# phaistos-networks/Trinity

Hardware: NVIDIA H100
Metric: queries/sec (batched 2-term AND, 100M-doc Zipfian synthetic index) (higher is better)
Workload: dtype u32

## Files before the change

### include/trinity_b200.h

```cpp
#ifndef TRINITY_B200_H
#define TRINITY_B200_H
#include <stddef.h>
#include <stdint.h>

#ifdef __cplusplus
extern "C" {
#endif

#define TRN_OK 0
#define TRN_ERR_ARG (-1)
#define TRN_ERR_CUDA (-2)
#define TRN_ERR_FORMAT (-3)
#define TRN_ERR_STATE (-4)
#define TRN_ERR_PARSE (-5)
#define TRN_ERR_CAPACITY (-6)
#define TRN_ERR_UNSUPPORTED (-7)

#define TRN_CODEC_GOOGLE 0
#define TRN_CODEC_LUCENE 1

typedef struct trn_term {
        uint32_t documents;
        uint32_t chunk_off;
        uint32_t chunk_len;
// ... 95 lines not shown

int         trn_create(int device, trn_ctx **out);
void        trn_destroy(trn_ctx *);
const char *trn_last_error(trn_ctx *);
int trn_set_stream(trn_ctx *, void *cuda_stream);

int trn_upload_index(trn_ctx *, int codec, const uint8_t *index, uint64_t nbytes, const trn_term *terms, uint32_t nterms, uint32_t max_docid);

int trn_set_masked_documents(trn_ctx *, const uint32_t *docids, uint64_t n);

typedef struct trn_index_info {
        int      codec;
        uint32_t nterms, max_docid, tile_docs, ntiles, block_docs;
        uint64_t index_bytes, directory_bytes, total_blocks, total_postings;
        uint64_t dense_terms, dense_bitmap_bytes;
} trn_index_info;
int trn_index_info_get(trn_ctx *, trn_index_info *out);

int trn_upload_hits(trn_ctx *, const uint8_t *index, uint64_t nbytes, const uint8_t *hits, uint64_t hits_bytes);

#define TRN_MODE_DOCS_ONLY 0
#define TRN_MODE_SCORED_ALL 1
#define TRN_MODE_SCORED_TOPK 2
#define TRN_MODE_DOCS_COMPACT 3

typedef struct trn_result {
        uint32_t        nq;
        uint64_t        total;
        const uint64_t *offsets;
        const uint32_t *docids;
// ... 43 lines not shown
#define TRN_ROUTE_CANDIDATE 3
#define TRN_ROUTE_SCORE_FLAT 4
#define TRN_ROUTE_FLAT_TREE 5
#define TRN_ROUTE_EXEC_TILES 6
int trn_debug_last_routes(trn_ctx *, uint8_t *out, uint32_t cap, uint32_t *n);
int trn_debug_plan(int codec, const uint8_t *index, uint64_t nbytes, const trn_term *terms, uint32_t nterms, uint32_t max_docid, const trn_query *queries,
                   uint32_t nq, int mode, uint32_t k, uint8_t *routes, uint32_t *nslots, char *err, size_t errcap);
int trn_debug_dense_runs(int codec, const uint8_t *index, uint64_t nbytes, const trn_term *terms, uint32_t nterms, uint32_t max_docid, const trn_query *queries,
                         uint32_t nq, int mode, uint32_t k, uint32_t *qtiles, uint32_t *tickets, uint64_t cap, uint64_t *n, char *err, size_t errcap);
int trn_debug_mixed_runs(int codec, const uint8_t *index, uint64_t nbytes, const trn_term *terms, uint32_t nterms, uint32_t max_docid, const trn_query *queries,
                         uint32_t nq, int mode, uint32_t k, uint32_t *qtiles, uint32_t *tickets, uint64_t cap, uint64_t *n, char *err, size_t errcap);
int trn_debug_cand_runs(int codec, const uint8_t *index, uint64_t nbytes, const trn_term *terms, uint32_t nterms, uint32_t max_docid, const trn_query *queries,
                        uint32_t nq, int mode, uint32_t k, uint32_t *qtiles, uint32_t *tickets, uint64_t cap, uint64_t *n, char *err, size_t errcap);

int trn_debug_dense_terms(int codec, const uint8_t *index, uint64_t nbytes, const trn_term *terms, uint32_t nterms, uint32_t *offsets, uint32_t *nselected,
                          uint64_t *bitmap_bytes, char *err, size_t errcap);

int trn_debug_dense_bitmap(trn_ctx *, uint32_t term, uint32_t *out, uint64_t cap, uint64_t *base, uint64_t *nwords);

#define TRN_MODE_MATCHED_TERMS 4
typedef struct trn_hit {
        uint64_t payload;
        uint16_t pos;
        uint8_t  payload_len;
} trn_hit;
typedef struct trn_matches {
        uint32_t        nq;
        uint64_t        total_matches, total_terms, total_hits;
        const uint64_t *doc_offsets;
        const uint32_t *docids;
// ... 163 lines not shown
```

### trinity_b200/__init__.py

```python
from __future__ import annotations

import ctypes as C
import os
from dataclasses import dataclass
from typing import Iterable, List, Optional, Sequence

import numpy as np

from ._ffi import (HIT_DTYPE, QNODE_DTYPE, TERM_DTYPE, TrnIndexInfo, TrnIntersections, TrnIsectReq, TrnMatches, TrnPercolation, TrnPercolatorInfo, TrnQuery,
                   TrnIndexed, TrnMerged, TrnMergeSource, TrnResult, TrnTerm, TrnTimings, lib)

CODEC_GOOGLE, CODEC_LUCENE = 0, 1
MODE_DOCS_ONLY, MODE_SCORED_ALL, MODE_SCORED_TOPK = 0, 1, 2
MODE_MATCHED_TERMS = 4
MODE_DOCS_COMPACT = 3
NODE_TERM, NODE_AND, NODE_OR, NODE_NOT, NODE_OPTIONAL, NODE_SOME, NODE_PHRASE = 0, 1, 2, 3, 4, 5, 6
ROUTE_STEPS, ROUTE_FLAT_AND, ROUTE_FLAT_OR, ROUTE_CANDIDATE, ROUTE_SCORE_FLAT, ROUTE_FLAT_TREE, ROUTE_EXEC_TILES = 0, 1, 2, 3, 4, 5, 6
EMPTY_TERM = 0xFFFFFFFF
DENSE_NONE = 0xFFFFFFFF
DOC_IDS_END = 0xFFFFFFFF
DOCSET_NONE = 0xFFFFFFFF


class TrinityError(RuntimeError):
# ... 277 lines not shown
    arr, keep = _pack_queries(queries)
    qtiles = np.zeros((max(len(queries), 1), 2), np.uint32)
    n = C.c_uint64()
    err = C.create_string_buffer(256)
    args = (codec, _ptr(index), index.size, _ptr(terms), len(terms), max_docid, C.cast(arr, C.c_void_p), len(queries), mode, k, _ptr(qtiles))
    rc = fn(*args, None, 0, C.byref(n), err, 256)
    tickets = np.zeros((max(n.value, 1), 3), np.uint32)
    if rc == -6:
        rc = fn(*args, _ptr(tickets), n.value, C.byref(n), err, 256)
    if rc != 0:
        raise TrinityError(err.value.decode("utf-8", "replace") or f"rc={rc}")
    return qtiles[: len(queries)].copy(), tickets[: n.value].copy()


def debug_dense_terms(codec: int, index: np.ndarray, terms: np.ndarray):
    index = np.ascontiguousarray(index, dtype=np.uint8)
    terms = np.ascontiguousarray(terms, dtype=TERM_DTYPE)
    off = np.zeros(max(len(terms), 1), np.uint32)
    n, nbytes = C.c_uint32(), C.c_uint64()
    err = C.create_string_buffer(256)
    rc = lib().trn_debug_dense_terms(codec, _ptr(index), index.size, _ptr(terms), len(terms), _ptr(off), C.byref(n), C.byref(nbytes), err, 256)
    if rc != 0:
        raise TrinityError(err.value.decode("utf-8", "replace") or f"rc={rc}")
    off = off[: len(terms)].copy()
    assert int(np.count_nonzero(off != DENSE_NONE)) == n.value
    return off, int(nbytes.value)


def bm25_idf(doc_freq: int, docs_cnt: int) -> float:
    return float(lib().trn_bm25_idf(doc_freq, docs_cnt))


def bm25_score(idf: float, freq: int) -> float:
    return float(lib().trn_bm25_score(idf, freq))


@dataclass
class BatchResult:
    nq: int
    mode: int
    k: int
# ... 788 lines not shown
```

### trinity_b200/_ffi.py

```python
from __future__ import annotations

import ctypes as C
from pathlib import Path

import numpy as np

_LIB_PATH = Path(__file__).resolve().parent / "libtrinity_b200.so"

EXPORTS = [
    "trn_builder_create", "trn_builder_destroy", "trn_builder_begin_term", "trn_builder_begin_document",
    "trn_builder_new_hit", "trn_builder_end_document", "trn_builder_end_term", "trn_builder_add_term",
    "trn_builder_set_google_skiplist_countdown", "trn_builder_index", "trn_builder_hits", "trn_builder_last_error",
    "trn_synth_build", "trn_synth_build_shard", "trn_synth_build_ex", "trn_builder_set_google_block", "trn_synth_destroy", "trn_synth_index", "trn_synth_hits", "trn_synth_terms", "trn_synth_sum_hits",
    "trn_synth_postings", "trn_synth_positions",
    "trn_directory_probe", "trn_directory_stats", "trn_directory_lookup", "trn_dict_create", "trn_dict_destroy", "trn_parse_query_dict", "trn_segment_open", "trn_segment_close", "trn_segment_info", "trn_segment_index", "trn_segment_terms",
    "trn_segment_masked", "trn_parse_query", "trn_query_truth_table", "trn_debug_compile", "trn_bm25_idf", "trn_bm25_score",
    "trn_create", "trn_destroy", "trn_last_error", "trn_set_stream", "trn_upload_index", "trn_set_masked_documents", "trn_index_info_get",
    "trn_exec_batch", "trn_exec_batch_device", "trn_last_topk_device", "trn_merge_topk", "trn_fetch_results", "trn_last_timings",
    "trn_decode_terms", "trn_result_for_each", "trn_result_decode", "trn_upload_hits", "trn_debug_positions", "trn_encode_google", "trn_encode_lucene", "trn_debug_chunk_plan",
    "trn_encode_google_payloads", "trn_encode_lucene_payloads", "trn_index_documents_payloads",
    "trn_debug_last_routes", "trn_debug_plan", "trn_debug_dense_runs", "trn_debug_mixed_runs", "trn_debug_cand_runs", "trn_debug_dense_terms", "trn_debug_dense_bitmap",
    "trn_exec_matches", "trn_debug_hits", "trn_intersect", "trn_debug_intersect_plan",
    "trn_percolator_register", "trn_percolate", "trn_debug_percolator_plan",
    "trn_index_documents", "trn_segment_write", "trn_merge_sources", "trn_merge_sources_payloads", "trn_debug_merge_plan",
    "trn_docset_create", "trn_docset_destroy", "trn_exec_batch_filtered", "trn_exec_batch_device_filtered", "trn_exec_matches_filtered",
]

TERM_DTYPE = np.dtype([("documents", "<u4"), ("chunk_off", "<u4"), ("chunk_len", "<u4")])
QNODE_DTYPE = np.dtype([("kind", "u1"), ("nchildren", "u1"), ("first_child", "<u2"), ("term", "<u4"), ("weight", "<f8")])
STEP_DTYPE = np.dtype([("op", "u1"), ("mode", "u1"), ("dst", "u1"), ("src", "u1"), ("flags", "u1"), ("pad", "u1", (3,)), ("term", "<u4"), ("pad2", "<u4"), ("idf", "<f8")])
assert TERM_DTYPE.itemsize == 12 and QNODE_DTYPE.itemsize == 16 and STEP_DTYPE.itemsize == 24


class TrnTerm(C.Structure):
    _fields_ = [("documents", C.c_uint32), ("chunk_off", C.c_uint32), ("chunk_len", C.c_uint32)]


class TrnQuery(C.Structure):
    _fields_ = [("nodes", C.c_void_p), ("nnodes", C.c_uint32), ("root", C.c_uint32)]


class TrnIndexInfo(C.Structure):
    _fields_ = [("codec", C.c_int), ("nterms", C.c_uint32), ("max_docid", C.c_uint32), ("tile_docs", C.c_uint32),
                ("ntiles", C.c_uint32), ("block_docs", C.c_uint32), ("index_bytes", C.c_uint64), ("directory_bytes", C.c_uint64),
                ("total_blocks", C.c_uint64), ("total_postings", C.c_uint64), ("dense_terms", C.c_uint64), ("dense_bitmap_bytes", C.c_uint64)]


class TrnResult(C.Structure):
    _fields_ = [("nq", C.c_uint32), ("total", C.c_uint64), ("offsets", C.POINTER(C.c_uint64)),
                ("docids", C.POINTER(C.c_uint32)), ("scores", C.POINTER(C.c_float)),
                ("match_counts", C.POINTER(C.c_uint64)), ("postings_scanned", C.c_uint64),
                ("index_bytes_touched", C.c_uint64), ("kernel_launches", C.c_uint32), ("device_ms", C.c_float), ("exec_kernel_ms", C.c_float),
                ("words", C.POINTER(C.c_uint32)), ("total_words", C.c_uint64), ("item_desc", C.POINTER(C.c_uint32)), ("qitems", C.c_void_p)]


HIT_DTYPE = np.dtype({"names": ["payload", "pos", "payload_len"], "formats": ["<u8", "<u2", "u1"], "offsets": [0, 8, 10], "itemsize": 16})


class TrnMatches(C.Structure):
    _fields_ = [("nq", C.c_uint32), ("total_matches", C.c_uint64), ("total_terms", C.c_uint64), ("total_hits", C.c_uint64),
# ... 138 lines not shown
    sig("trn_encode_lucene_payloads", i32, vp, vp, u32, vp, vp, vp, vp, vp, vp, C.c_uint64, P(C.c_uint64), vp, C.c_uint64, P(C.c_uint64), vp, P(C.c_float))
    sig("trn_debug_last_routes", i32, vp, vp, u32, P(u32))
    sig("trn_exec_matches", i32, vp, vp, u32, P(TrnMatches))
    sig("trn_docset_create", i32, vp, vp, u64, P(u32))
    sig("trn_docset_destroy", i32, vp, u32)
    sig("trn_exec_batch_filtered", i32, vp, vp, u32, i32, u32, vp, P(TrnResult))
    sig("trn_exec_batch_device_filtered", i32, vp, vp, u32, i32, u32, vp, P(TrnResult))
    sig("trn_exec_matches_filtered", i32, vp, vp, u32, vp, P(TrnMatches))
    sig("trn_debug_hits", i32, i32, vp, C.c_uint64, vp, C.c_uint64, vp, vp, u32, vp, vp, vp, C.c_uint64, P(C.c_uint64), C.c_char_p, C.c_size_t)
    sig("trn_debug_plan", i32, i32, vp, u64, vp, u32, u32, vp, u32, i32, u32, vp, P(u32), C.c_char_p, C.c_size_t)
    sig("trn_debug_dense_runs", i32, i32, vp, u64, vp, u32, u32, vp, u32, i32, u32, vp, vp, u64, P(u64), C.c_char_p, C.c_size_t)
    sig("trn_debug_mixed_runs", i32, i32, vp, u64, vp, u32, u32, vp, u32, i32, u32, vp, vp, u64, P(u64), C.c_char_p, C.c_size_t)
    sig("trn_debug_cand_runs", i32, i32, vp, u64, vp, u32, u32, vp, u32, i32, u32, vp, vp, u64, P(u64), C.c_char_p, C.c_size_t)
    sig("trn_debug_dense_bitmap", i32, vp, u32, vp, u64, P(u64), P(u64))
    sig("trn_debug_dense_terms", i32, i32, vp, u64, vp, u32, vp, P(u32), P(u64), C.c_char_p, C.c_size_t)
    sig("trn_intersect", i32, vp, vp, u32, P(TrnIntersections))
    sig("trn_debug_intersect_plan", i32, vp, vp, u32, u32, vp, vp, vp, vp, u64, P(u32), P(u64), vp, P(u32), C.c_char_p, C.c_size_t)
    sig("trn_percolator_register", i32, vp, vp, u32, u32, vp, P(TrnPercolatorInfo))
    sig("trn_percolate", i32, vp, vp, vp, u32, P(TrnPercolation))
    sig("trn_debug_percolator_plan", i32, vp, u32, u32, vp, vp, vp, vp, u64, P(u64), C.c_char_p, C.c_size_t)
    sig("trn_index_documents", i32, vp, i32, vp, vp, vp, vp, u32, u32, P(TrnIndexed))
    sig("trn_index_documents_payloads", i32, vp, i32, vp, vp, vp, vp, vp, vp, u32, u32, P(TrnIndexed))
    sig("trn_segment_write", i32, C.c_char_p, i32, vp, u64, vp, u64, vp, vp, u32, u64, u32, u64, u32, vp, u64, C.c_char_p, C.c_size_t)
    sig("trn_merge_sources", i32, vp, i32, vp, u32, i32, P(TrnMerged))
    sig("trn_merge_sources_payloads", i32, vp, i32, vp, u32, i32, P(TrnMerged))
    sig("trn_debug_merge_plan", i32, i32, vp, u32, i32, vp, vp, vp, vp, vp, vp, P(u32), P(u64), vp, vp, P(u64), P(u32), C.c_char_p, C.c_size_t)
    _lib = L
    return L
```

### trinity_b200/csrc/device_types.h

```cpp
#pragma once
#include "../../include/trinity_b200.h"
#include <cstdint>
#include <vector_types.h>

namespace trn {

struct HitTerm;

static constexpr uint32_t kEmptyTerm = 0xffffffffu;
static constexpr uint32_t kDenseAlignShift = 17;
static constexpr uint32_t kDenseNone       = 0xffffffffu;

__host__ __device__ inline uint32_t dense_run_end(uint32_t first, uint32_t tile_lo, uint32_t ntiles, uint32_t exec_shift) {
        const uint32_t e = (first | ((1u << (kDenseAlignShift - exec_shift)) - 1u)) + 1u, qe = tile_lo + ntiles;
        return e < qe ? e : qe;
}

struct DevTerm {
        uint32_t documents;
        uint32_t dir_begin;
        uint32_t nblocks;
        uint32_t first_doc;
        uint32_t last_doc;
        uint32_t chunk_len;
// ... 10 lines not shown
        const DevTerm * terms;
        const uint32_t *masked;
        const uint32_t *tile_first;
        uint32_t        nterms;
        uint32_t        ntiles;
        uint32_t        tile_shift;
        uint32_t        max_docid;
        uint32_t        block_docs;
        int             codec;
        const uint8_t * hits;
        const uint32_t *hit_base;
        const uint32_t *hblk_off;
        const struct HitTerm *hit_term;
        const uint32_t *dense;
        const uint32_t *dense_off;
};

enum StepOp : uint8_t {
        OP_LEAF      = 0,
        OP_SLOT      = 1,
        OP_CLEAR     = 2,
        OP_LEAFSCORE = 3,
        OP_COUNT_ADD = 4,
        OP_COUNT_GE  = 5,
        OP_PHRASE    = 7,
        OP_ARG       = 8,
        OP_TABLE     = 6,
};
enum StepMode : uint8_t { M_SET = 0, M_OR = 1, M_AND = 2, M_ANDNOT = 3, M_NONE = 4 };
static constexpr uint32_t kEncU32 = 0, kEncU16 = 1, kEncBitmap = 2, kEncU8B = 3;
// ... 340 lines not shown
```

### trinity_b200/csrc/engine.cu

```cuda
#include "../../include/trinity_b200.h"
#include "codecs.h"
#include "device_types.h"
#include "hitcursor.h"
#include "chunkplan.h"
#include "isectplan.h"
#include "percplan.h"
#include "mergeplan.h"
#include "kernels.h"
#include "planner.h"
#include <algorithm>
#include <array>
#include <chrono>
#include <cmath>
#include <cstdio>
#include <cstdlib>
#include <cstring>
#include <limits>
#include <stdexcept>
#include <functional>
#include <map>
#include <string>
#include <unordered_map>
#include <thread>
#include <vector>
// ... 69 lines not shown
        DevBuf               d_index, d_blk_last, d_blk_off, d_terms, d_tile_first, d_masked;
        bool                 have_masked{false};
        struct DocSet {
                DevBuf   bits;
                uint32_t lo{1}, hi{0};
                bool     live{false};
        };
        std::vector<DocSet> docsets;
        uint32_t            docset_epoch{0};
        uint32_t            docset_max{0xffffu};
        DevBuf              d_filters;
        DevBuf               d_dense, d_dense_off;
        uint32_t             dense_terms{0};
        uint64_t             dense_bytes{0};
        std::vector<uint32_t> h_dense_off;
        std::vector<DevTerm> h_terms;
        GroupStarts          h_groups;
        DevBuf d_queries, d_steps, d_dense_runs, d_mixed_runs, d_cand_order, d_small[2], d_item_off, d_item_cnt, d_item_dst, d_seg_docids, d_seg_scores, d_out_docids[2], d_out_scores[2], d_q_offsets[2], d_cand,
            d_topk_docids, d_topk_scores, d_topk_counts, d_fq, d_leaves, d_luts, d_dec_units, d_dec_c, d_dec_docids, d_dec_freqs, d_dec_sums, d_merge_docids, d_merge_scores;
        PinBuf h_offsets, h_docids, h_scores, h_counts, h_small, h_chunk, h_item_desc;
        DevBuf d_hits, d_hit_base, d_hblk_off, d_hit_term;
        bool   have_hits{false};
        BlockDirectory              h_dir;
        std::vector<term_index_ctx> h_termctx;
        DevBuf d_item_desc[2];
        std::vector<trn_qitems> qitems_set[2];
        std::vector<trn_qitems> h_qitems;
        std::vector<std::vector<trn_qitems>> qitems_chunk;
        uint64_t                last_items_hint{0};
        cudaEvent_t ev0{nullptr}, ev1{nullptr}, evk0{nullptr}, evk1{nullptr};
// ... 180 lines not shown
        for (int i = 0; i < 16; ++i) {
                CK(cudaEventCreate(&c->ev_ck0[i]));
                CK(cudaEventCreate(&c->ev_ck1[i]));
        }
        CK(cudaEventCreate(&c->ev0));
        CK(cudaEventCreate(&c->ev1));
        CK(cudaEventCreate(&c->evk0));
        CK(cudaEventCreate(&c->evk1));
        return TRN_OK;
}

extern "C" void trn_destroy(trn_ctx *c) {
        if (!c)
                return;
        cudaSetDevice(c->device);
        for (DevBuf *b : {&c->d_index, &c->d_blk_last, &c->d_blk_off, &c->d_terms, &c->d_tile_first, &c->d_masked, &c->d_dense, &c->d_dense_off, &c->d_queries, &c->d_steps, &c->d_dense_runs, &c->d_mixed_runs, &c->d_cand_order, &c->d_small[0], &c->d_small[1], &c->d_item_off,
                          &c->d_item_cnt, &c->d_item_dst, &c->d_seg_docids, &c->d_seg_scores, &c->d_out_docids[0], &c->d_out_docids[1], &c->d_out_scores[0], &c->d_out_scores[1], &c->d_q_offsets[0], &c->d_q_offsets[1], &c->d_cand,
                          &c->d_topk_docids, &c->d_topk_scores, &c->d_topk_counts, &c->d_fq, &c->d_leaves, &c->d_luts, &c->d_dec_units, &c->d_dec_c, &c->d_dec_docids, &c->d_dec_freqs,
                          &c->d_dec_sums, &c->d_merge_docids, &c->d_merge_scores, &c->d_filters})
                b->release();
        for (auto &d : c->docsets)
                d.bits.release();
        for (PinBuf *b : {&c->h_offsets, &c->h_docids, &c->h_scores, &c->h_counts, &c->h_small, &c->h_chunk, &c->h_item_desc})
                b->release();
        for (cudaEvent_t e : {c->ev0, c->ev1, c->evk0, c->evk1, c->ev_done[0], c->ev_done[1], c->ev_d2h[0], c->ev_d2h[1]})
                if (e)
                        cudaEventDestroy(e);
        for (int i = 0; i < 16; ++i) {
                if (c->ev_ck0[i])
                        cudaEventDestroy(c->ev_ck0[i]);
                if (c->ev_ck1[i])
// ... 11 lines not shown

extern "C" const char *trn_last_error(trn_ctx *c) {
        return c ? c->err.c_str() : "null ctx";
}

extern "C" int trn_set_stream(trn_ctx *c, void *s) {
        if (!c)
                return TRN_ERR_ARG;
        c->stream = static_cast<cudaStream_t>(s);
        return TRN_OK;
}

static int upload_dense(trn_ctx *c) {
        c->dense_terms = 0;
        c->dense_bytes = 0;
        c->h_dense_off.clear();
        DenseSelection                  s;
        std::vector<unsigned long long> prefix;
        try {
                s = select_dense_terms(c->pc, c->h_terms, c->index_bytes);
                prefix.assign(s.order.size() + 1, 0ull);
                for (size_t i = 0; i < s.order.size(); ++i)
                        prefix[i + 1] = prefix[i] + c->h_terms[s.order[i]].nblocks;
        } catch (const std::bad_alloc &) {
                s = DenseSelection{};
                c->err = "dense-term bitmaps off for this index: out of host memory";
        }
        DevBuf sel, pre;
        cudaError_t e = cudaSuccess;
        if (!s.order.empty()) {
                e = c->d_dense.ensure(s.words * 4);
                if (e == cudaSuccess)
                        e = c->d_dense_off.ensure(std::max<size_t>(4, s.off.size() * 4));
                if (e == cudaSuccess)
                        e = sel.ensure(s.order.size() * 4);
                if (e == cudaSuccess)
                        e = pre.ensure(prefix.size() * 8);
        }
        if (s.order.empty() || e != cudaSuccess) {
                if (e != cudaSuccess) {
                        (void)cudaGetLastError();
                        c->err = std::string("dense-term bitmaps off for this index: ") + cudaGetErrorString(e);
                }
                c->d_dense.release();
                c->d_dense_off.release();
                sel.release();
                pre.release();
                return TRN_OK;
        }
        CK(cudaMemsetAsync(c->d_dense.p, 0, s.words * 4, c->stream));
        CK(cudaMemcpyAsync(c->d_dense_off.p, s.off.data(), s.off.size() * 4, cudaMemcpyHostToDevice, c->stream));
        CK(cudaMemcpyAsync(sel.p, s.order.data(), s.order.size() * 4, cudaMemcpyHostToDevice, c->stream));
        CK(cudaMemcpyAsync(pre.p, prefix.data(), prefix.size() * 8, cudaMemcpyHostToDevice, c->stream));
        c->dense_terms = uint32_t(s.order.size());
        (void)cudaGetLastError();
        const cudaError_t le = launch_build_dense(dev_index(c), sel.as<uint32_t>(), pre.as<unsigned long long>(), uint32_t(s.order.size()), prefix.back(),
                                                  c->d_dense.as<uint32_t>(), c->stream);
        const cudaError_t se = cudaStreamSynchronize(c->stream);
        sel.release();
        pre.release();
        if (le != cudaSuccess || se != cudaSuccess) {
                c->dense_terms = 0;
                return fail(c, TRN_ERR_CUDA, std::string("building the dense-term bitmaps: ") + cudaGetErrorString(le != cudaSuccess ? le : se));
        }
        c->dense_bytes = s.words * 4;
        c->h_dense_off = std::move(s.off);
        return TRN_OK;
}

static void drop_docsets(trn_ctx *c) {
        for (auto &d : c->docsets)
                d.bits.release();
        c->docsets.clear();
        ++c->docset_epoch;
}

extern "C" int trn_upload_index(trn_ctx *c, int codec, const uint8_t *index, uint64_t nbytes, const trn_term *terms, uint32_t nterms, uint32_t max_docid) {
        if (!c || !index || !terms || (codec != TRN_CODEC_GOOGLE && codec != TRN_CODEC_LUCENE))
                return c ? fail(c, TRN_ERR_ARG, "trn_upload_index: bad arguments") : TRN_ERR_ARG;
        if (nbytes >= (1ull << 32))
// ... 266 lines not shown
                return TRN_ERR_ARG;
        if (!c->have_index)
                return fail(c, TRN_ERR_STATE, "no index uploaded");
        o->codec           = c->pc.codec;
        o->nterms          = c->nterms;
        o->max_docid       = c->pc.max_docid;
        o->tile_docs       = 1u << c->pc.tile_shift;
        o->ntiles          = c->ntiles;
        o->block_docs      = c->block_docs;
        o->index_bytes     = c->index_bytes;
        o->directory_bytes = c->dir_bytes;
        o->total_blocks    = c->total_blocks;
        o->total_postings  = c->total_postings;
        o->dense_terms        = c->dense_terms;
        o->dense_bitmap_bytes = c->dense_bytes;
        return TRN_OK;
}

static DevIndex dev_index(trn_ctx *c) {
        DevIndex ix;
        ix.index      = c->d_index.as<uint8_t>();
        ix.blk_last   = c->d_blk_last.as<uint32_t>();
        ix.blk_off    = c->d_blk_off.as<uint32_t>();
        ix.terms      = c->d_terms.as<DevTerm>();
        ix.tile_first = c->d_tile_first.as<uint32_t>();
        ix.masked     = c->have_masked ? c->d_masked.as<uint32_t>() : nullptr;
        ix.nterms     = c->nterms;
        ix.ntiles     = c->ntiles;
        ix.tile_shift = c->pc.tile_shift;
        ix.max_docid  = c->pc.max_docid;
        ix.block_docs = c->block_docs;
        ix.codec      = c->pc.codec;
        ix.hits       = c->have_hits ? c->d_hits.as<uint8_t>() : nullptr;
        ix.hit_base   = c->have_hits ? c->d_hit_base.as<uint32_t>() : nullptr;
        ix.hblk_off   = c->have_hits ? c->d_hblk_off.as<uint32_t>() : nullptr;
        ix.hit_term   = c->have_hits ? c->d_hit_term.as<HitTerm>() : nullptr;
        ix.dense      = c->dense_terms ? c->d_dense.as<uint32_t>() : nullptr;
        ix.dense_off  = c->dense_terms ? c->d_dense_off.as<uint32_t>() : nullptr;
        return ix;
}

static int exec_device_impl(trn_ctx *c, const trn_query *queries, uint32_t nq, int mode, uint32_t k, trn_result *out, int set, cudaEvent_t k0, cudaEvent_t k1,
                            uint8_t *routes, const trn_doc_filter *filters, CollectPlan *collect = nullptr) {
        if (!c)
                return TRN_ERR_ARG;
        if (!c->have_index)
                return fail(c, TRN_ERR_STATE, "no index uploaded");
        if (!queries || !nq || mode < 0 || mode > 3)
                return fail(c, TRN_ERR_ARG, "trn_exec_batch: bad arguments");
        const bool compact = mode == TRN_MODE_DOCS_COMPACT;
        if (compact)
                mode = TRN_MODE_DOCS_ONLY;
        if (c->block_docs != (c->pc.codec == TRN_CODEC_GOOGLE ? 32u : 128u))
// ... 876 lines not shown
        return debug_run_tickets(RunTickets::dense, codec, index, nbytes, terms, nterms, max_docid, queries, nq, mode, k, qtiles, tickets, cap, n, err, errcap);
}

extern "C" int trn_debug_mixed_runs(int codec, const uint8_t *index, uint64_t nbytes, const trn_term *terms, uint32_t nterms, uint32_t max_docid,
                                    const trn_query *queries, uint32_t nq, int mode, uint32_t k, uint32_t *qtiles, uint32_t *tickets, uint64_t cap, uint64_t *n,
                                    char *err, size_t errcap) {
        return debug_run_tickets(RunTickets::mixed, codec, index, nbytes, terms, nterms, max_docid, queries, nq, mode, k, qtiles, tickets, cap, n, err, errcap);
}

extern "C" int trn_debug_cand_runs(int codec, const uint8_t *index, uint64_t nbytes, const trn_term *terms, uint32_t nterms, uint32_t max_docid,
                                   const trn_query *queries, uint32_t nq, int mode, uint32_t k, uint32_t *qtiles, uint32_t *tickets, uint64_t cap, uint64_t *n,
                                   char *err, size_t errcap) {
        return debug_run_tickets(RunTickets::cand, codec, index, nbytes, terms, nterms, max_docid, queries, nq, mode, k, qtiles, tickets, cap, n, err, errcap);
}

extern "C" int trn_debug_dense_terms(int codec, const uint8_t *index, uint64_t nbytes, const trn_term *terms, uint32_t nterms, uint32_t *offsets,
                                     uint32_t *nselected, uint64_t *bitmap_bytes, char *err, size_t errcap) {
        auto seterr = [&](const std::string &m, int rc) {
                if (err && errcap) {
                        std::strncpy(err, m.c_str(), errcap - 1);
                        err[errcap - 1] = 0;
                }
                return rc;
        };
        if (!index || !terms || (nterms && !offsets) || !nselected || !bitmap_bytes || (codec != TRN_CODEC_GOOGLE && codec != TRN_CODEC_LUCENE))
                return seterr("bad arguments", TRN_ERR_ARG);
        DenseSelection s;
        try {
                BlockDirectory dir;
                build_directory(codec, index, nbytes, terms, nterms, 1, dir);
                PlanConfig pc = initial_plan_config();
                pc.codec      = codec;
                s             = select_dense_terms(pc, dev_terms(dir, terms, nterms), nbytes);
        } catch (const std::exception &e) {
                return seterr(e.what(), TRN_ERR_FORMAT);
        }
        if (nterms)
                std::memcpy(offsets, s.off.data(), nterms * 4);
        *nselected    = uint32_t(s.order.size());
        *bitmap_bytes = s.words * 4;
        return TRN_OK;
}

extern "C" int trn_debug_dense_bitmap(trn_ctx *c, uint32_t term, uint32_t *out, uint64_t cap, uint64_t *base, uint64_t *nwords) {
        if (!c || !base || !nwords)
                return TRN_ERR_ARG;
        if (!c->have_index)
                return fail(c, TRN_ERR_STATE, "no index uploaded");
        if (term >= c->nterms)
                return fail(c, TRN_ERR_ARG, "trn_debug_dense_bitmap: no such term");
        *base   = 0;
        *nwords = 0;
        if (!c->dense_terms || c->h_dense_off[term] == kDenseNone)
                return TRN_OK;
        dense_span(c->h_terms[term], *base, *nwords);
        if (cap < *nwords || !out)
// ... 1780 lines not shown
```

### trinity_b200/csrc/exec_docs_cand.cuh

```cuda
#pragma once

static constexpr uint32_t kCandStride  = 33;
static constexpr uint32_t kCandWords   = 32 * kCandStride;
static constexpr uint32_t kCandBytes   = kCandWords * 4;
static constexpr uint32_t kCandMaskBytes = kCandWords;
static constexpr uint32_t kCandSmem    = kCandBytes + kGatherBufBytes;
static constexpr uint32_t kCandSmemMask = kCandSmem + kCandMaskBytes;
static constexpr uint32_t kCandInvalid = 0xffffffffu;
static constexpr uint32_t kCandProbeRounds = 2;
static_assert(32u % kCandProbeRounds == 0, "a group's 32 rounds split into whole batches");

__device__ __forceinline__ void google_block_to_array(const uint8_t *__restrict__ index, uint32_t off, const uint8_t *buf, int lane, uint32_t n, uint32_t prev,
                                                      uint32_t last, uint32_t *out) {
        const uint32_t mis = off & 15u;
        const uint32_t sp  = uint32_t(__cvta_generic_to_shared(buf + lane * kGatherBytes)) + mis;
        const uint32_t nd  = n - 1u;
        uint32_t       doc = prev, i = 0, p = 0;
        bool           live = true;
#pragma unroll 1
        for (uint32_t it = 0; it < 31u; ++it) {
                const uint32_t at = sp + p, a = at & ~3u;
                const uint32_t w  = __funnelshift_r(lds_u32(a), lds_u32(a + 4u), (at & 3u) * 8u);
                const uint32_t b0 = w & 0xffu;
                const uint32_t two = b0 >= 0x80u ? 1u : 0u, three = b0 >= 0xc0u ? 1u : 0u;
// ... 77 lines not shown
                                myTerm = st.term;
                        ++nleaf;
                } else if (st.op == OP_TABLE) {
                        const unsigned long long hi = static_cast<unsigned long long>(__double_as_longlong(st.idf));
                        const uint32_t           w  = uint32_t(lane) - st.dst;
                        if (w == 0u) myTable = st.term;
                        else if (w == 1u) myTable = st.pad2;
                        else if (w == 2u) myTable = uint32_t(hi);
                        else if (w == 3u) myTable = uint32_t(hi >> 32);
                }
        }
        const uint32_t nnec = Q.root_slot;
        uint32_t mydir = 0, mynb = 0, mydocs = 0, myfirst = 0, mylast = 0, mytfb = 0, mytfbase = 0, mytfs = 32, mydense = kDenseNone;
        if (uint32_t(lane) < nleaf && myTerm != kEmptyTerm) {
                const DevTerm T = P.ix.terms[myTerm];
                if (P.ix.dense_off)
                        mydense = __ldg(P.ix.dense_off + myTerm);
                mydir           = T.dir_begin;
                mynb            = T.nblocks;
                mydocs          = T.documents;
                myfirst         = T.first_doc;
                mylast          = T.last_doc;
                mytfb           = T.tf_begin;
                mytfbase        = T.tf_base;
                mytfs           = T.tf_shift;
        }
        const uint32_t dir0 = __shfl_sync(0xffffffffu, mydir, 0), nb0 = __shfl_sync(0xffffffffu, mynb, 0), docs0 = __shfl_sync(0xffffffffu, mydocs, 0);
        DevFilter      F{};
        if constexpr (FILT) {
                F = P.filters[curq];
                const uint32_t b0 = group * 32u, b1 = min(nb0, b0 + 32u);
                const bool     out = b0 >= b1 || F.lo > F.hi || __ldg(P.ix.blk_last + dir0 + b1 - 1u) < F.lo || (b0 && __ldg(P.ix.blk_last + dir0 + b0 - 1u) >= F.hi);
// ... 171 lines not shown
```

### trinity_b200/csrc/kernels.cu

```cuda
#include "device_types.h"
#include "dirlookup.h"
#include "hitcursor.h"
#include "kernels.h"
#include "varbyte.h"
#include <algorithm>
#include <type_traits>
#include <cuda_runtime.h>

namespace trn {

static constexpr int      kThreads    = 128;
static constexpr int      kWarps      = kThreads / 32;
static constexpr uint32_t kStageBytes = 6144;
static constexpr uint32_t kListCap    = 2048;
static constexpr uint32_t kTileListCap = 1024;
static constexpr uint32_t kMaxK       = 512;

__device__ __forceinline__ uint4 ld_stream_v4(const void *p) {
        uint4 r;
        asm volatile("ld.global.nc.L1::no_allocate.v4.u32 {%0,%1,%2,%3}, [%4];" : "=r"(r.x), "=r"(r.y), "=r"(r.z), "=r"(r.w) : "l"(p));
        return r;
}

__device__ __forceinline__ uint32_t warp_incl_scan(uint32_t v, int lane) {
// ... 938 lines not shown
__global__ void __launch_bounds__(kThreads) k_build_dense(DevIndex ix, const uint32_t *sel, const unsigned long long *blk_prefix, uint32_t nsel,
                                                           unsigned long long total_blocks, uint32_t *dense) {
        const unsigned long long g = blockIdx.x * 1ull * blockDim.x + threadIdx.x;
        if (g >= total_blocks)
                return;
        uint32_t lo = 0, hi = nsel;
        while (hi - lo > 1u) {
                const uint32_t mid = (lo + hi) >> 1;
                if (blk_prefix[mid] <= g) lo = mid;
                else hi = mid;
        }
        const uint32_t  t = sel[lo], b = uint32_t(g - blk_prefix[lo]);
        const DevTerm   T = ix.terms[t];
        const uint32_t *bl = ix.blk_last + T.dir_begin;
        const uint32_t  base = (T.first_doc >> kDenseAlignShift) << kDenseAlignShift;
        uint32_t *      bm   = dense + ix.dense_off[t];
        const uint32_t  n    = (b + 1u == T.nblocks) ? (T.documents - 32u * (T.nblocks - 1u)) : 32u;
        const uint8_t * p    = ix.index + ix.blk_off[T.dir_begin + b];
        uint32_t        doc = b ? bl[b - 1] : 0u, cw = 0xffffffffu, cur = 0;
        for (uint32_t i = 0; i < n; ++i) {
                doc               = i + 1u < n ? doc + varbyte_get(p) : bl[b];
                const uint32_t w  = (doc - base) >> 5;
                if (w != cw && cur)
                        atomicOr(bm + cw, cur);
                cur = (w != cw ? 0u : cur) | (1u << (doc & 31u));
                cw  = w;
        }
        if (cur)
                atomicOr(bm + cw, cur);
}

// ... 15 lines not shown
```

### trinity_b200/csrc/planner.cpp

```cpp
#include "planner.h"
#include <algorithm>
#include <cmath>
#include <cstdlib>
#include <cstring>

using namespace trn;

namespace {
struct Range {
        uint32_t lo{1}, hi{0};
        bool     empty() const {
                return lo > hi;
        }
};

static bool plan_is_tree(const trn_qnode *n, uint32_t nn, uint32_t root) {
        std::vector<uint8_t> seen(nn, 0);
        if (root < nn)
                seen[root] = 1;
        for (uint32_t i = 0; i < nn; ++i) {
                if (n[i].kind == TRN_NODE_TERM)
                        continue;
                for (uint32_t k = 0; k < n[i].nchildren; ++k) {
                        const uint32_t c = uint32_t(n[i].first_child) + k;
// ... 870 lines not shown
        }
        if (const char *e = getenv("TRN_FLAT_SCORED"))
                pc.flat_scored = atoi(e) != 0;
        if (const char *e = getenv("TRN_SCORED_SHIFT")) {
                const int v = atoi(e);
                if (v == 13 || v == 14)
                        pc.scored_shift = uint32_t(v);
        }
        if (const char *e = getenv("TRN_DENSE_BITMAPS"))
                pc.dense_bitmaps = atoi(e) != 0;
        if (const char *e = getenv("TRN_DENSE_BUDGET")) {
                const double v = atof(e);
                if (v >= 0.0 && v <= 1.0)
                        pc.dense_budget = v;
        }
        if (const char *e = getenv("TRN_DENSE_RUNS"))
                pc.dense_runs = atoi(e) != 0;
        if (const char *e = getenv("TRN_MIXED_RUNS"))
                pc.mixed_runs = atoi(e) != 0;
        if (const char *e = getenv("TRN_CAND_RUNS"))
                pc.cand_runs = atoi(e) != 0;
        return pc;
}

trn::GroupStarts trn::group_starts(const BlockDirectory &dir) {
        GroupStarts g;
        g.base.resize(dir.terms.size());
        uint64_t n{0};
        for (size_t t = 0; t < dir.terms.size(); ++t) {
                g.base[t] = uint32_t(n);
// ... 22 lines not shown
        std::vector<uint32_t> cand;
        for (uint32_t t = 0; t < terms.size(); ++t) {
                uint64_t base, words;
                dense_span(terms[t], base, words);
                if (terms[t].nblocks && words * 4 <= terms[t].chunk_len)
                        cand.push_back(t);
        }
        std::stable_sort(cand.begin(), cand.end(), [&](uint32_t a, uint32_t b) { return terms[a].documents > terms[b].documents; });
        const double budget = cfg.dense_budget * double(index_bytes);
        for (uint32_t t : cand) {
                uint64_t base, words;
                dense_span(terms[t], base, words);
                if (double((s.words + words) * 4) > budget)
                        break;
                s.off[t] = uint32_t(s.words);
                s.order.push_back(t);
                s.words += words;
        }
        return s;
}

void trn::build_directory(int codec, const uint8_t *index, uint64_t nbytes, const trn_term *terms, uint32_t nterms, int threads, BlockDirectory &dir) {
        std::vector<term_index_ctx> t(nterms);
        for (uint32_t i = 0; i < nterms; ++i) {
                t[i].documents = terms[i].documents;
                t[i].offset    = terms[i].chunk_off;
                t[i].size      = terms[i].chunk_len;
        }
        build_block_directory(codec == TRN_CODEC_GOOGLE ? Codec::Google : Codec::Lucene, index, nbytes, t.data(), nterms, threads, dir);
}
// ... 481 lines not shown
```

### trinity_b200/csrc/planner.h

```cpp
#pragma once
#include "../../include/trinity_b200.h"
#include "codecs.h"
#include "device_types.h"
#include <string>
#include <vector>

namespace trn {

struct PlanConfig {
        int      codec{0};
        uint32_t min_docid{1};
        uint32_t max_docid{0};
        uint32_t tile_shift{13};
        uint32_t docs_shift{14};
        uint32_t tree_shift{13};
        uint32_t scored_shift{13};
        uint32_t run_tiles{128};
        int      cand_cost{900};
        bool     flat_scored{true};
        bool     allow_phrase{false};
        bool     dense_bitmaps{true};
        double   dense_budget{0.25};
        bool     dense_runs{true};
        bool     mixed_runs{true};
        bool     cand_runs{true};
        uint32_t score_flat_max_leaves{0};
        uint32_t docs_stage_bytes{0};
        uint32_t cand_smem_bytes[2]{0, 0};
        uint32_t mixed_smem_bytes{0};
};

PlanConfig plan_config_from_env();

struct BatchPlan {
        std::vector<DevQuery>  queries;
        std::vector<DevStep>   steps;
        std::vector<FlatQuery> flat;
// ... 30 lines not shown
        std::vector<uint32_t> base;
        std::vector<uint32_t> first;
};
GroupStarts group_starts(const BlockDirectory &dir);
int plan_batch(const PlanConfig &cfg, const std::vector<DevTerm> &terms, const uint32_t *dense_off, const trn_query *queries, uint32_t nq, int mode,
               uint32_t k, BatchPlan &out, std::string &err, const uint2 *clip = nullptr, const GroupStarts *groups = nullptr);

struct DenseSelection {
        std::vector<uint32_t> off;
        std::vector<uint32_t> order;
        uint64_t              words{0};
};
void dense_span(const DevTerm &T, uint64_t &base, uint64_t &words);
DenseSelection select_dense_terms(const PlanConfig &cfg, const std::vector<DevTerm> &terms, uint64_t index_bytes);

void build_directory(int codec, const uint8_t *index, uint64_t nbytes, const trn_term *terms, uint32_t nterms, int threads, BlockDirectory &dir);
std::vector<DevTerm> dev_terms(const BlockDirectory &dir, const trn_term *terms, uint32_t nterms);
void docid_span(const std::vector<DevTerm> &terms, uint32_t &min_docid, uint32_t &max_docid);

}
```

Baseline: 108,100.

## Add probe bitmaps for mid-frequency terms used by candidate AND path

Beyond the dense-term bitmaps, a second set of terms is selected whose docid bitmap span is at most a ratio of their compressed chunk size, up to a budget of twice the index size. These bitmaps are built alongside the dense ones, and the candidate AND kernel looks them up through a new probe offset table. Candidate checks can then test membership in a bitmap instead of decoding posting blocks. The cost is considerably more device memory and longer index upload, and bitmaps are disabled when the block size is not the Google codec's.

```diff
diff --git a/include/trinity_b200.h b/include/trinity_b200.h
--- a/include/trinity_b200.h
+++ b/include/trinity_b200.h
@@ -133,6 +133,7 @@
         uint32_t nterms, max_docid, tile_docs, ntiles, block_docs;
         uint64_t index_bytes, directory_bytes, total_blocks, total_postings;
         uint64_t dense_terms, dense_bitmap_bytes;
+        uint64_t probe_terms, probe_bitmap_bytes;
 } trn_index_info;
 int trn_index_info_get(trn_ctx *, trn_index_info *out);
 
@@ -206,6 +207,9 @@
                         uint32_t nq, int mode, uint32_t k, uint32_t *qtiles, uint32_t *tickets, uint64_t cap, uint64_t *n, char *err, size_t errcap);
 
 int trn_debug_dense_terms(int codec, const uint8_t *index, uint64_t nbytes, const trn_term *terms, uint32_t nterms, uint32_t *offsets, uint32_t *nselected,
+                          uint64_t *bitmap_bytes, char *err, size_t errcap);
+
+int trn_debug_probe_terms(int codec, const uint8_t *index, uint64_t nbytes, const trn_term *terms, uint32_t nterms, uint32_t *offsets, uint32_t *nselected,
                           uint64_t *bitmap_bytes, char *err, size_t errcap);
 
 int trn_debug_dense_bitmap(trn_ctx *, uint32_t term, uint32_t *out, uint64_t cap, uint64_t *base, uint64_t *nwords);
diff --git a/trinity_b200/__init__.py b/trinity_b200/__init__.py
--- a/trinity_b200/__init__.py
+++ b/trinity_b200/__init__.py
@@ -315,17 +315,25 @@
 
 
 def debug_dense_terms(codec: int, index: np.ndarray, terms: np.ndarray):
+    off, n, nbytes = _debug_bitmap_terms(lib().trn_debug_dense_terms, codec, index, terms)
+    assert int(np.count_nonzero(off != DENSE_NONE)) == n
+    return off, nbytes
+
+
+def debug_probe_terms(codec: int, index: np.ndarray, terms: np.ndarray):
+    return _debug_bitmap_terms(lib().trn_debug_probe_terms, codec, index, terms)
+
+
+def _debug_bitmap_terms(fn, codec, index, terms):
     index = np.ascontiguousarray(index, dtype=np.uint8)
     terms = np.ascontiguousarray(terms, dtype=TERM_DTYPE)
     off = np.zeros(max(len(terms), 1), np.uint32)
     n, nbytes = C.c_uint32(), C.c_uint64()
     err = C.create_string_buffer(256)
-    rc = lib().trn_debug_dense_terms(codec, _ptr(index), index.size, _ptr(terms), len(terms), _ptr(off), C.byref(n), C.byref(nbytes), err, 256)
+    rc = fn(codec, _ptr(index), index.size, _ptr(terms), len(terms), _ptr(off), C.byref(n), C.byref(nbytes), err, 256)
     if rc != 0:
         raise TrinityError(err.value.decode("utf-8", "replace") or f"rc={rc}")
-    off = off[: len(terms)].copy()
-    assert int(np.count_nonzero(off != DENSE_NONE)) == n.value
-    return off, int(nbytes.value)
+    return off[: len(terms)].copy(), n.value, int(nbytes.value)
 
 
 def bm25_idf(doc_freq: int, docs_cnt: int) -> float:
diff --git a/trinity_b200/_ffi.py b/trinity_b200/_ffi.py
--- a/trinity_b200/_ffi.py
+++ b/trinity_b200/_ffi.py
@@ -19,7 +19,7 @@
     "trn_exec_batch", "trn_exec_batch_device", "trn_last_topk_device", "trn_merge_topk", "trn_fetch_results", "trn_last_timings",
     "trn_decode_terms", "trn_result_for_each", "trn_result_decode", "trn_upload_hits", "trn_debug_positions", "trn_encode_google", "trn_encode_lucene", "trn_debug_chunk_plan",
     "trn_encode_google_payloads", "trn_encode_lucene_payloads", "trn_index_documents_payloads",
-    "trn_debug_last_routes", "trn_debug_plan", "trn_debug_dense_runs", "trn_debug_mixed_runs", "trn_debug_cand_runs", "trn_debug_dense_terms", "trn_debug_dense_bitmap",
+    "trn_debug_last_routes", "trn_debug_plan", "trn_debug_dense_runs", "trn_debug_mixed_runs", "trn_debug_cand_runs", "trn_debug_dense_terms", "trn_debug_probe_terms", "trn_debug_dense_bitmap",
     "trn_exec_matches", "trn_debug_hits", "trn_intersect", "trn_debug_intersect_plan",
     "trn_percolator_register", "trn_percolate", "trn_debug_percolator_plan",
     "trn_index_documents", "trn_segment_write", "trn_merge_sources", "trn_merge_sources_payloads", "trn_debug_merge_plan",
@@ -43,7 +43,8 @@
 class TrnIndexInfo(C.Structure):
     _fields_ = [("codec", C.c_int), ("nterms", C.c_uint32), ("max_docid", C.c_uint32), ("tile_docs", C.c_uint32),
                 ("ntiles", C.c_uint32), ("block_docs", C.c_uint32), ("index_bytes", C.c_uint64), ("directory_bytes", C.c_uint64),
-                ("total_blocks", C.c_uint64), ("total_postings", C.c_uint64), ("dense_terms", C.c_uint64), ("dense_bitmap_bytes", C.c_uint64)]
+                ("total_blocks", C.c_uint64), ("total_postings", C.c_uint64), ("dense_terms", C.c_uint64), ("dense_bitmap_bytes", C.c_uint64),
+                ("probe_terms", C.c_uint64), ("probe_bitmap_bytes", C.c_uint64)]
 
 
 class TrnResult(C.Structure):
@@ -212,6 +213,7 @@
     sig("trn_debug_cand_runs", i32, i32, vp, u64, vp, u32, u32, vp, u32, i32, u32, vp, vp, u64, P(u64), C.c_char_p, C.c_size_t)
     sig("trn_debug_dense_bitmap", i32, vp, u32, vp, u64, P(u64), P(u64))
     sig("trn_debug_dense_terms", i32, i32, vp, u64, vp, u32, vp, P(u32), P(u64), C.c_char_p, C.c_size_t)
+    sig("trn_debug_probe_terms", i32, i32, vp, u64, vp, u32, vp, P(u32), P(u64), C.c_char_p, C.c_size_t)
     sig("trn_intersect", i32, vp, vp, u32, P(TrnIntersections))
     sig("trn_debug_intersect_plan", i32, vp, vp, u32, u32, vp, vp, vp, vp, u64, P(u32), P(u64), vp, P(u32), C.c_char_p, C.c_size_t)
     sig("trn_percolator_register", i32, vp, vp, u32, u32, vp, P(TrnPercolatorInfo))
diff --git a/trinity_b200/csrc/device_types.h b/trinity_b200/csrc/device_types.h
--- a/trinity_b200/csrc/device_types.h
+++ b/trinity_b200/csrc/device_types.h
@@ -48,6 +48,7 @@
         const struct HitTerm *hit_term;
         const uint32_t *dense;
         const uint32_t *dense_off;
+        const uint32_t *probe_off;
 };
 
 enum StepOp : uint8_t {
diff --git a/trinity_b200/csrc/engine.cu b/trinity_b200/csrc/engine.cu
--- a/trinity_b200/csrc/engine.cu
+++ b/trinity_b200/csrc/engine.cu
@@ -107,6 +107,9 @@
         uint32_t             dense_terms{0};
         uint64_t             dense_bytes{0};
         std::vector<uint32_t> h_dense_off;
+        DevBuf               d_probe_off;
+        uint32_t             probe_terms{0};
+        uint64_t             probe_bytes{0};
         std::vector<DevTerm> h_terms;
         GroupStarts          h_groups;
         DevBuf d_queries, d_steps, d_dense_runs, d_mixed_runs, d_cand_order, d_small[2], d_item_off, d_item_cnt, d_item_dst, d_seg_docids, d_seg_scores, d_out_docids[2], d_out_scores[2], d_q_offsets[2], d_cand,
@@ -317,7 +320,7 @@
         if (!c)
                 return;
         cudaSetDevice(c->device);
-        for (DevBuf *b : {&c->d_index, &c->d_blk_last, &c->d_blk_off, &c->d_terms, &c->d_tile_first, &c->d_masked, &c->d_dense, &c->d_dense_off, &c->d_queries, &c->d_steps, &c->d_dense_runs, &c->d_mixed_runs, &c->d_cand_order, &c->d_small[0], &c->d_small[1], &c->d_item_off,
+        for (DevBuf *b : {&c->d_index, &c->d_blk_last, &c->d_blk_off, &c->d_terms, &c->d_tile_first, &c->d_masked, &c->d_dense, &c->d_dense_off, &c->d_probe_off, &c->d_queries, &c->d_steps, &c->d_dense_runs, &c->d_mixed_runs, &c->d_cand_order, &c->d_small[0], &c->d_small[1], &c->d_item_off,
                           &c->d_item_cnt, &c->d_item_dst, &c->d_seg_docids, &c->d_seg_scores, &c->d_out_docids[0], &c->d_out_docids[1], &c->d_out_scores[0], &c->d_out_scores[1], &c->d_q_offsets[0], &c->d_q_offsets[1], &c->d_cand,
                           &c->d_topk_docids, &c->d_topk_scores, &c->d_topk_counts, &c->d_fq, &c->d_leaves, &c->d_luts, &c->d_dec_units, &c->d_dec_c, &c->d_dec_docids, &c->d_dec_freqs,
                           &c->d_dec_sums, &c->d_merge_docids, &c->d_merge_scores, &c->d_filters})
@@ -359,56 +362,95 @@
 static int upload_dense(trn_ctx *c) {
         c->dense_terms = 0;
         c->dense_bytes = 0;
+        c->probe_terms = 0;
+        c->probe_bytes = 0;
         c->h_dense_off.clear();
-        DenseSelection                  s;
-        std::vector<unsigned long long> prefix;
+        DenseSelection s, p;
         try {
                 s = select_dense_terms(c->pc, c->h_terms, c->index_bytes);
-                prefix.assign(s.order.size() + 1, 0ull);
-                for (size_t i = 0; i < s.order.size(); ++i)
-                        prefix[i + 1] = prefix[i] + c->h_terms[s.order[i]].nblocks;
+                p = select_probe_terms(c->pc, c->h_terms, c->index_bytes, s);
         } catch (const std::bad_alloc &) {
-                s = DenseSelection{};
+                s = p = DenseSelection{};
                 c->err = "dense-term bitmaps off for this index: out of host memory";
         }
-        DevBuf sel, pre;
+        if (c->block_docs != Codecs::Google::N)
+                s = p = DenseSelection{};
+        DevBuf      sel, pre;
         cudaError_t e = cudaSuccess;
-        if (!s.order.empty()) {
-                e = c->d_dense.ensure(s.words * 4);
+        auto        allocate = [&] {
+                const size_t nsel = s.order.size() + p.order.size();
+                e                 = c->d_dense.ensure((s.words + p.words) * 4);
                 if (e == cudaSuccess)
                         e = c->d_dense_off.ensure(std::max<size_t>(4, s.off.size() * 4));
                 if (e == cudaSuccess)
-                        e = sel.ensure(s.order.size() * 4);
+                        e = c->d_probe_off.ensure(std::max<size_t>(4, p.off.size() * 4));
                 if (e == cudaSuccess)
-                        e = pre.ensure(prefix.size() * 8);
-        }
-        if (s.order.empty() || e != cudaSuccess) {
+                        e = sel.ensure(nsel * 4);
+                if (e == cudaSuccess)
+                        e = pre.ensure((nsel + 1) * 8);
                 if (e != cudaSuccess) {
                         (void)cudaGetLastError();
+                        for (DevBuf *b : {&c->d_dense, &c->d_dense_off, &c->d_probe_off, &sel, &pre})
+                                b->release();
+                }
+        };
+        if (!p.order.empty()) {
+                allocate();
+                if (e != cudaSuccess) {
+                        c->err          = std::string("probe bitmaps off for this index: ") + cudaGetErrorString(e);
+                        p.order.clear();
+                        p.words         = 0;
+                        p.off           = s.off;
+                        e               = cudaSuccess;
+                }
+        }
+        if (p.order.empty() && !s.order.empty()) {
+                allocate();
+                if (e != cudaSuccess)
                         c->err = std::string("dense-term bitmaps off for this index: ") + cudaGetErrorString(e);
-                }
+        }
+        std::vector<uint32_t>           order;
+        std::vector<unsigned long long> prefix;
+        if (e == cudaSuccess) {
+                try {
+                        order = s.order;
+                        order.insert(order.end(), p.order.begin(), p.order.end());
+                        prefix.assign(order.size() + 1, 0ull);
+                        for (size_t i = 0; i < order.size(); ++i)
+                                prefix[i + 1] = prefix[i] + c->h_terms[order[i]].nblocks;
+                } catch (const std::bad_alloc &) {
+                        order.clear();
+                        c->err = "dense-term bitmaps off for this index: out of host memory";
+                }
+        }
+        if (order.empty()) {
                 c->d_dense.release();
                 c->d_dense_off.release();
+                c->d_probe_off.release();
                 sel.release();
                 pre.release();
                 return TRN_OK;
         }
-        CK(cudaMemsetAsync(c->d_dense.p, 0, s.words * 4, c->stream));
+        CK(cudaMemsetAsync(c->d_dense.p, 0, (s.words + p.words) * 4, c->stream));
         CK(cudaMemcpyAsync(c->d_dense_off.p, s.off.data(), s.off.size() * 4, cudaMemcpyHostToDevice, c->stream));
-        CK(cudaMemcpyAsync(sel.p, s.order.data(), s.order.size() * 4, cudaMemcpyHostToDevice, c->stream));
+        CK(cudaMemcpyAsync(c->d_probe_off.p, p.off.data(), p.off.size() * 4, cudaMemcpyHostToDevice, c->stream));
+        CK(cudaMemcpyAsync(sel.p, order.data(), order.size() * 4, cudaMemcpyHostToDevice, c->stream));
         CK(cudaMemcpyAsync(pre.p, prefix.data(), prefix.size() * 8, cudaMemcpyHostToDevice, c->stream));
         c->dense_terms = uint32_t(s.order.size());
+        c->probe_terms = uint32_t(p.order.size());
         (void)cudaGetLastError();
-        const cudaError_t le = launch_build_dense(dev_index(c), sel.as<uint32_t>(), pre.as<unsigned long long>(), uint32_t(s.order.size()), prefix.back(),
+        const cudaError_t le = launch_build_dense(dev_index(c), sel.as<uint32_t>(), pre.as<unsigned long long>(), uint32_t(order.size()), prefix.back(),
                                                   c->d_dense.as<uint32_t>(), c->stream);
         const cudaError_t se = cudaStreamSynchronize(c->stream);
         sel.release();
         pre.release();
         if (le != cudaSuccess || se != cudaSuccess) {
                 c->dense_terms = 0;
+                c->probe_terms = 0;
                 return fail(c, TRN_ERR_CUDA, std::string("building the dense-term bitmaps: ") + cudaGetErrorString(le != cudaSuccess ? le : se));
         }
         c->dense_bytes = s.words * 4;
+        c->probe_bytes = p.words * 4;
         c->h_dense_off = std::move(s.off);
         return TRN_OK;
 }
@@ -705,6 +747,8 @@
         o->total_postings  = c->total_postings;
         o->dense_terms        = c->dense_terms;
         o->dense_bitmap_bytes = c->dense_bytes;
+        o->probe_terms        = c->probe_terms;
+        o->probe_bitmap_bytes = c->probe_bytes;
         return TRN_OK;
 }
 
@@ -726,8 +770,10 @@
         ix.hit_base   = c->have_hits ? c->d_hit_base.as<uint32_t>() : nullptr;
         ix.hblk_off   = c->have_hits ? c->d_hblk_off.as<uint32_t>() : nullptr;
         ix.hit_term   = c->have_hits ? c->d_hit_term.as<HitTerm>() : nullptr;
-        ix.dense      = c->dense_terms ? c->d_dense.as<uint32_t>() : nullptr;
+        const bool bitmaps = c->dense_terms || c->probe_terms;
+        ix.dense      = bitmaps ? c->d_dense.as<uint32_t>() : nullptr;
         ix.dense_off  = c->dense_terms ? c->d_dense_off.as<uint32_t>() : nullptr;
+        ix.probe_off  = bitmaps ? c->d_probe_off.as<uint32_t>() : nullptr;
         return ix;
 }
 
@@ -1634,8 +1680,8 @@
         return debug_run_tickets(RunTickets::cand, codec, index, nbytes, terms, nterms, max_docid, queries, nq, mode, k, qtiles, tickets, cap, n, err, errcap);
 }
 
-extern "C" int trn_debug_dense_terms(int codec, const uint8_t *index, uint64_t nbytes, const trn_term *terms, uint32_t nterms, uint32_t *offsets,
-                                     uint32_t *nselected, uint64_t *bitmap_bytes, char *err, size_t errcap) {
+static int debug_bitmap_terms(bool probe, int codec, const uint8_t *index, uint64_t nbytes, const trn_term *terms, uint32_t nterms, uint32_t *offsets,
+                              uint32_t *nselected, uint64_t *bitmap_bytes, char *err, size_t errcap) {
         auto seterr = [&](const std::string &m, int rc) {
                 if (err && errcap) {
                         std::strncpy(err, m.c_str(), errcap - 1);
@@ -1651,7 +1697,10 @@
                 build_directory(codec, index, nbytes, terms, nterms, 1, dir);
                 PlanConfig pc = initial_plan_config();
                 pc.codec      = codec;
-                s             = select_dense_terms(pc, dev_terms(dir, terms, nterms), nbytes);
+                const std::vector<DevTerm> ht = dev_terms(dir, terms, nterms);
+                s                             = select_dense_terms(pc, ht, nbytes);
+                if (probe)
+                        s = select_probe_terms(pc, ht, nbytes, s);
         } catch (const std::exception &e) {
                 return seterr(e.what(), TRN_ERR_FORMAT);
         }
@@ -1660,6 +1709,16 @@
         *nselected    = uint32_t(s.order.size());
         *bitmap_bytes = s.words * 4;
         return TRN_OK;
+}
+
+extern "C" int trn_debug_dense_terms(int codec, const uint8_t *index, uint64_t nbytes, const trn_term *terms, uint32_t nterms, uint32_t *offsets,
+                                     uint32_t *nselected, uint64_t *bitmap_bytes, char *err, size_t errcap) {
+        return debug_bitmap_terms(false, codec, index, nbytes, terms, nterms, offsets, nselected, bitmap_bytes, err, errcap);
+}
+
+extern "C" int trn_debug_probe_terms(int codec, const uint8_t *index, uint64_t nbytes, const trn_term *terms, uint32_t nterms, uint32_t *offsets,
+                                     uint32_t *nselected, uint64_t *bitmap_bytes, char *err, size_t errcap) {
+        return debug_bitmap_terms(true, codec, index, nbytes, terms, nterms, offsets, nselected, bitmap_bytes, err, errcap);
 }
 
 extern "C" int trn_debug_dense_bitmap(trn_ctx *c, uint32_t term, uint32_t *out, uint64_t cap, uint64_t *base, uint64_t *nwords) {
diff --git a/trinity_b200/csrc/exec_docs_cand.cuh b/trinity_b200/csrc/exec_docs_cand.cuh
--- a/trinity_b200/csrc/exec_docs_cand.cuh
+++ b/trinity_b200/csrc/exec_docs_cand.cuh
@@ -115,8 +115,8 @@
         uint32_t mydir = 0, mynb = 0, mydocs = 0, myfirst = 0, mylast = 0, mytfb = 0, mytfbase = 0, mytfs = 32, mydense = kDenseNone;
         if (uint32_t(lane) < nleaf && myTerm != kEmptyTerm) {
                 const DevTerm T = P.ix.terms[myTerm];
-                if (P.ix.dense_off)
-                        mydense = __ldg(P.ix.dense_off + myTerm);
+                if (P.ix.probe_off)
+                        mydense = __ldg(P.ix.probe_off + myTerm);
                 mydir           = T.dir_begin;
                 mynb            = T.nblocks;
                 mydocs          = T.documents;
diff --git a/trinity_b200/csrc/kernels.cu b/trinity_b200/csrc/kernels.cu
--- a/trinity_b200/csrc/kernels.cu
+++ b/trinity_b200/csrc/kernels.cu
@@ -976,7 +976,7 @@
         const DevTerm   T = ix.terms[t];
         const uint32_t *bl = ix.blk_last + T.dir_begin;
         const uint32_t  base = (T.first_doc >> kDenseAlignShift) << kDenseAlignShift;
-        uint32_t *      bm   = dense + ix.dense_off[t];
+        uint32_t *      bm   = dense + ix.probe_off[t];
         const uint32_t  n    = (b + 1u == T.nblocks) ? (T.documents - 32u * (T.nblocks - 1u)) : 32u;
         const uint8_t * p    = ix.index + ix.blk_off[T.dir_begin + b];
         uint32_t        doc = b ? bl[b - 1] : 0u, cw = 0xffffffffu, cur = 0;
diff --git a/trinity_b200/csrc/planner.cpp b/trinity_b200/csrc/planner.cpp
--- a/trinity_b200/csrc/planner.cpp
+++ b/trinity_b200/csrc/planner.cpp
@@ -908,6 +908,18 @@
                 if (v >= 0.0 && v <= 1.0)
                         pc.dense_budget = v;
         }
+        if (const char *e = getenv("TRN_PROBE_BITMAPS"))
+                pc.probe_bitmaps = atoi(e) != 0;
+        if (const char *e = getenv("TRN_PROBE_RATIO")) {
+                const double v = atof(e);
+                if (v > 0.0)
+                        pc.probe_ratio = v;
+        }
+        if (const char *e = getenv("TRN_PROBE_BUDGET")) {
+                const double v = atof(e);
+                if (v >= 0.0)
+                        pc.probe_budget = v;
+        }
         if (const char *e = getenv("TRN_DENSE_RUNS"))
                 pc.dense_runs = atoi(e) != 0;
         if (const char *e = getenv("TRN_MIXED_RUNS"))
@@ -960,6 +972,32 @@
                 if (double((s.words + words) * 4) > budget)
                         break;
                 s.off[t] = uint32_t(s.words);
+                s.order.push_back(t);
+                s.words += words;
+        }
+        return s;
+}
+
+trn::DenseSelection trn::select_probe_terms(const PlanConfig &cfg, const std::vector<DevTerm> &terms, uint64_t index_bytes, const DenseSelection &dense) {
+        DenseSelection s;
+        s.off = dense.off;
+        if (cfg.codec != TRN_CODEC_GOOGLE || !cfg.dense_bitmaps || !cfg.probe_bitmaps)
+                return s;
+        std::vector<uint32_t> cand;
+        for (uint32_t t = 0; t < terms.size(); ++t) {
+                uint64_t base, words;
+                dense_span(terms[t], base, words);
+                if (terms[t].nblocks && dense.off[t] == kDenseNone && double(words * 4) <= cfg.probe_ratio * double(terms[t].chunk_len))
+                        cand.push_back(t);
+        }
+        std::stable_sort(cand.begin(), cand.end(), [&](uint32_t a, uint32_t b) { return terms[a].documents > terms[b].documents; });
+        const double budget = cfg.probe_budget * double(index_bytes);
+        for (uint32_t t : cand) {
+                uint64_t base, words;
+                dense_span(terms[t], base, words);
+                if (double((s.words + words) * 4) > budget || dense.words + s.words + words >= (1ull << 32))
+                        break;
+                s.off[t] = uint32_t(dense.words + s.words);
                 s.order.push_back(t);
                 s.words += words;
         }
diff --git a/trinity_b200/csrc/planner.h b/trinity_b200/csrc/planner.h
--- a/trinity_b200/csrc/planner.h
+++ b/trinity_b200/csrc/planner.h
@@ -21,6 +21,9 @@
         bool     allow_phrase{false};
         bool     dense_bitmaps{true};
         double   dense_budget{0.25};
+        bool     probe_bitmaps{true};
+        double   probe_ratio{16.0};
+        double   probe_budget{2.0};
         bool     dense_runs{true};
         bool     mixed_runs{true};
         bool     cand_runs{true};
@@ -81,6 +84,8 @@
 void dense_span(const DevTerm &T, uint64_t &base, uint64_t &words);
 DenseSelection select_dense_terms(const PlanConfig &cfg, const std::vector<DevTerm> &terms, uint64_t index_bytes);
 
+DenseSelection select_probe_terms(const PlanConfig &cfg, const std::vector<DevTerm> &terms, uint64_t index_bytes, const DenseSelection &dense);
+
 void build_directory(int codec, const uint8_t *index, uint64_t nbytes, const trn_term *terms, uint32_t nterms, int threads, BlockDirectory &dir);
 std::vector<DevTerm> dev_terms(const BlockDirectory &dir, const trn_term *terms, uint32_t nterms);
 void docid_span(const std::vector<DevTerm> &terms, uint32_t &min_docid, uint32_t &max_docid);
```

Measured after the change: 129,500, median of 6. +19.8%, better.
